# PieterBecking/so100-mujoco-rl

Measured on AMD Instinct MI355X. Metric: env steps/sec at 4096 envs/GPU, Env01 PPO rollout, higher is better.
Workload: dtype f32; 1 GPU; env01_free: Env01 x 4096 envs/GPU, frame_skip 16, contact disabled, no constraint solver (BASELINE.json configs[1]), SB3-MlpPolicy-shaped rollout (persistent policy), randomized resets, staggered episodes; envs_per_gpu=4096, rollout_chunk=64, parallelism=single GPU

## Files before the change

so100_mujoco_rl_amd/csrc/so100_kernels.hpp:

```cpp
#pragma once
#include <hip/hip_runtime.h>
#include <stdint.h>
#include <stdio.h>
#include <string.h>
#include <stdlib.h>
#include <new>
#include "../../include/so100_sim.h"
#include "so100_task.hpp"
#include "so100_policy.hpp"

namespace so100 {
template <int KIND, int FL = -1> __device__ __forceinline__ void load_env_state(const float* __restrict__ S, int n, int env, EnvState& e) {
#define X(name, member, kind, group) \
    if constexpr (uses_group<KIND, FL>(group)) { const float w_ = S[(size_t)SF_##name*n + env]; \
        if constexpr (#kind[0] == 'i') e.member = __float_as_int(w_); else e.member = w_; }
    SO100_STATE_FIELDS(X)
#undef X
}
template <typename M> __device__ __forceinline__ float as_word(M v) {
    if constexpr (sizeof(M) == 4 && !__is_floating_point(M)) return __int_as_float((int)v); else return (float)v;
}
template <int KIND, int FL = -1> __device__ __forceinline__ void store_env_state(float* __restrict__ S, int n, int env, const EnvState& e) {
#define X(name, member, kind, group) \
    if constexpr (uses_group<KIND, FL>(group)) S[(size_t)SF_##name*n + env] = as_word(e.member);
// ... 38 lines not shown
    store_env_state<KIND, FL>(io.state, p.n, env, e);
#pragma unroll
    for (int i = 0; i < OD; i++) io.obs[(size_t)env*OD + i] = obs[i];
    io.rew[env] = r.reward;
    if (io.rollout_row) {
        io.rollout_row[(size_t)env*(OD + ROW_EXTRA) + OD + ROW_REWARD] = r.reward;
        io.rollout_row[(size_t)env*(OD + ROW_EXTRA) + OD + ROW_DONE] = done_code(r.done, r.trunc_only);
    }
    io.done[env] = r.done ? 1 : 0;
    io.trunc[env] = r.trunc_only ? 1 : 0;
    if (r.done) {
        if (io.tobs) {
#pragma unroll
            for (int i = 0; i < OD; i++) io.tobs[(size_t)env*OD + i] = tobs[i];
        }
        if (io.ep_ret) io.ep_ret[env] = r.ep_return;
        if (io.ep_len) io.ep_len[env] = r.ep_length;
    }
}

template <int KIND, int FL>
__global__ void __launch_bounds__(256) so100_step_mw(SimParams p, StepPtrs io) {
    constexpr bool PADS = FL < 0 || (FL & (int)F_ANY_CONTACT) != 0;
    constexpr bool LINKS = FL < 0 || (FL & (int)F_ANY_LINKS) != 0;
    __shared__ float xq[PADS ? 24 : 18][64];
    __shared__ float xc[24][64];
    __shared__ float xb[6][64];
    __shared__ float cbuf[PADS ? MAXC*CF*64 : 1];
    __shared__ float xa[PADS ? 15 : 1][64];
    __shared__ float xk[PADS ? 12 : 1][64];
    __shared__ float xm[PADS ? 21 : 1][64];
    __shared__ unsigned char pbuf[PADS ? MAXC*64 : 1];
    __shared__ float xw[PADS ? 36 : 1][64];
    if (FL >= 0) p.flags = (unsigned)FL;
    const int lane = threadIdx.x & 63;
    const int wave = __builtin_amdgcn_readfirstlane(threadIdx.x >> 6);
    const int env = blockIdx.x*p.epw + lane;
    const bool live = lane < p.epw && env < p.n;
    constexpr int OD = obs_dim<KIND>();
    EnvState e; StepCtx ctx{}; float u[8] = {}; float cstale[3] = {};
    const float* inj = (io.inject && live) ? io.inject + (size_t)env*SO100_NINJECT : nullptr;
    if (wave == 0) {
        if (live) load_env_state<KIND, FL>(io.state, p.n, env, e); else idle_lane_state(e);
        float a[6];
#pragma unroll
        for (int i = 0; i < 6; i++) a[i] = live ? io.act[(size_t)env*6 + i] : 0.0f;
        draw8(p, p.env_id_offset + (uint32_t)env, (uint32_t)e.rngc, 0, inj, u);
        e.rngc++;
        env_step_pre<KIND>(e, a, u, p, ctx);
    }
    Arm<float> A; Prof prof_;
    const PhaseLds lds{ xq, xc, xb, cbuf, xa, xk, xm, pbuf, PADS ? xw : nullptr };
    ContactMemo memo;
    physics_phase_mw<PADS, LINKS, !PADS && FL != 7, !PADS && FL != 7, !PADS && FL != 7>(p, wave, lane, e, ctx.ctrl, cstale, A, lds, memo, prof_, [](int) {}, [&]() {
        ctx = StepCtx{};
#pragma unroll
        for (int k = 0; k < 8; k++) u[k] = 0.0f;
    });
    if (wave != 0 || !live) return;
    e.nsub += p.frame_skip;
    TaskPoses<float> P;
    task_poses<float, !PADS && FL != 7>(A.s, A.c, !reach_kind<KIND>(), P);
    float obs[OD], tobs[OD]; bool term;
    const float reward = env_step_post<KIND>(e, ctx, u, P, cstale, obs, term);
    const StepResult r = env_step_finish<KIND>(e, reward, term, p, p.env_id_offset + (uint32_t)env, inj, io.start_tab, obs, tobs);
    if constexpr (PADS) e.cload &= 0xFFFF;
    store_env_state<KIND, FL>(io.state, p.n, env, e);
#pragma unroll
    for (int i = 0; i < OD; i++) io.obs[(size_t)env*OD + i] = obs[i];
    io.rew[env] = r.reward;
    if (io.rollout_row) {
        io.rollout_row[(size_t)env*(OD + ROW_EXTRA) + OD + ROW_REWARD] = r.reward;
        io.rollout_row[(size_t)env*(OD + ROW_EXTRA) + OD + ROW_DONE] = done_code(r.done, r.trunc_only);
    }
    io.done[env] = r.done ? 1 : 0;
    io.trunc[env] = r.trunc_only ? 1 : 0;
    if (r.done) {
        if (io.tobs) {
#pragma unroll
            for (int i = 0; i < OD; i++) io.tobs[(size_t)env*OD + i] = tobs[i];
        }
        if (io.ep_ret) io.ep_ret[env] = r.ep_return;
        if (io.ep_len) io.ep_len[env] = r.ep_length;
    }
}

template <int KIND>
__global__ void __launch_bounds__(WG) so100_reset_masked(SimParams p, float* state, const float* start_tab,
                                                         const uint8_t* mask, const float* inject, float* obs_out) {
    const int env = blockIdx.x*WG + threadIdx.x;
    if (env >= p.n) return;
    if (mask && !mask[env]) return;
    EnvState e;
    load_env_state<KIND>(state, p.n, env, e);
    float u[8];
    const float* inj = inject ? inject + (size_t)env*SO100_NINJECT : nullptr;
    draw8(p, p.env_id_offset + (uint32_t)env, (uint32_t)e.rngc, 1, inj, u);
    e.rngc++;
    constexpr int OD = obs_dim<KIND>();
    float obs[OD];
    env_reset<KIND>(e, u, start_tab, obs);
    store_env_state<KIND>(state, p.n, env, e);
    if (obs_out) {
#pragma unroll
        for (int i = 0; i < OD; i++) obs_out[(size_t)env*OD + i] = obs[i];
    }
}

template <int KIND>
__global__ void __launch_bounds__(WG) so100_init_state(int n, float* state) {
    const int env = blockIdx.x*WG + threadIdx.x;
    if (env >= n) return;
    for (int f = 0; f < SF_COUNT; f++) state[(size_t)f*n + env] = 0.0f;
    EnvState e;
    env_init<KIND>(e);
    store_env_state<KIND>(state, n, env, e);
}


constexpr int MW_MAX_ENVS = 16384;
inline dim3 grid_for(int n) { return dim3((unsigned)((n + WG - 1)/WG)); }

struct RolloutPtrs { float* obs; float* rew; uint8_t* done; uint8_t* trunc; float* tobs; float* ep_ret; int32_t* ep_len; };

template <int KIND> struct KindOps {
    static hipError_t step(const SimParams& prm, const StepPtrs& io, hipStream_t st);
    static hipError_t reset(const SimParams& prm, float* state, const float* start_tab, const uint8_t* mask, const float* inject, float* obs, hipStream_t st);
    static hipError_t init(int n, float* state);
    static hipError_t rollout(const SimParams& prm, float* state, const float* start_tab, const RolloutPtrs& io, const PolicyWeights& pw, const RolloutArgs& ra, hipStream_t st);
#ifdef SO100_ROLLOUT_PROF
    static int prof_read(long long* out48);
    static int prof_read_wg(long long* wg4096, int* env32768);
    static int prof_read_hist(unsigned long long* hist48, int reset);
#endif
};
#ifdef SO100_ROLLOUT_PROF
template <int KIND> int KindOps<KIND>::prof_read(long long* out48) {
    return hipMemcpyFromSymbol(out48, HIP_SYMBOL(so100_prof), sizeof(long long)*48) == hipSuccess ? 0 : -1;
}
template <int KIND> int KindOps<KIND>::prof_read_hist(unsigned long long* h, int reset) {
    if (hipMemcpyFromSymbol(h, HIP_SYMBOL(so100_prof_hist), sizeof(unsigned long long)*48) != hipSuccess) return -1;
    if (reset) { unsigned long long z[48] = {}; if (hipMemcpyToSymbol(HIP_SYMBOL(so100_prof_hist), z, sizeof z) != hipSuccess) return -1; }
    return 0;
}
template <int KIND> int KindOps<KIND>::prof_read_wg(long long* wg, int* env) {
    if (hipMemcpyFromSymbol(wg, HIP_SYMBOL(so100_prof_wg), sizeof(long long)*4096) != hipSuccess) return -1;
    return hipMemcpyFromSymbol(env, HIP_SYMBOL(so100_prof_env), sizeof(int)*32768) == hipSuccess ? 0 : -1;
}
#endif

template <int KIND> hipError_t KindOps<KIND>::step(const SimParams& prm, const StepPtrs& io, hipStream_t st) {
    const bool mw = prm.n <= prm.mw_max;
    const dim3 g = mw ? dim3((unsigned)((prm.n + prm.epw - 1)/prm.epw)) : grid_for(prm.n), b(mw ? 256 : WG);
#define SO100_STEP(FLV) do { if (mw) hipLaunchKernelGGL((so100_step_mw<KIND, FLV>), g, b, 0, st, prm, io); \
                             else    hipLaunchKernelGGL((so100_step_fused<KIND, FLV>), g, b, 0, st, prm, io); } while (0)
#define SO100_STEP_ROWS(FLV) do { if (!mw && prm.n >= DENSE_MIN_ENVS) hipLaunchKernelGGL((so100_step_fused<KIND, FLV, true>), g, b, 0, st, prm, io); \
                                  else SO100_STEP(FLV); } while (0)
    switch (prm.flags) {
    case SO100_F_CUBE_PINNED: SO100_STEP(SO100_F_CUBE_PINNED); break;
    case SO100_F_FRICTIONLOSS | SO100_F_LIMITS | SO100_F_CUBE_PINNED: SO100_STEP_ROWS(SO100_F_FRICTIONLOSS | SO100_F_LIMITS | SO100_F_CUBE_PINNED); break;
    case SO100_F_NOPADS: SO100_STEP_ROWS(SO100_F_NOPADS); break;
    case SO100_F_REFERENCE: SO100_STEP(SO100_F_REFERENCE); break;
    case SO100_F_CONTACT5: if constexpr (reach_kind<KIND>()) { SO100_STEP(SO100_F_CONTACT5); } else { SO100_STEP(-1); } break;
    default: SO100_STEP(-1); break;
    }
#undef SO100_STEP_ROWS
#undef SO100_STEP
    return hipGetLastError();
}
template <int KIND> hipError_t KindOps<KIND>::reset(const SimParams& prm, float* state, const float* start_tab, const uint8_t* mask, const float* inject, float* obs, hipStream_t st) {
    hipLaunchKernelGGL(so100_reset_masked<KIND>, grid_for(prm.n), dim3(WG), 0, st, prm, state, start_tab, mask, inject, obs);
    return hipGetLastError();
}
template <int KIND> hipError_t KindOps<KIND>::init(int n, float* state) {
    hipLaunchKernelGGL(so100_init_state<KIND>, grid_for(n), dim3(WG), 0, nullptr, n, state);
    const hipError_t e = hipGetLastError();
    return e != hipSuccess ? e : hipDeviceSynchronize();
}
template <int KIND> hipError_t KindOps<KIND>::rollout(const SimParams& prm, float* state, const float* start_tab, const RolloutPtrs& io, const PolicyWeights& pw, const RolloutArgs& ra, hipStream_t st) {
    const dim3 grid((unsigned)((prm.n + prm.epw - 1)/prm.epw));
#define SO100_RL(FLV) hipLaunchKernelGGL((so100_rollout_fused<KIND, FLV, 4>), grid, dim3(256), 0, st, prm, state, start_tab, \
        io.obs, io.rew, io.done, io.trunc, io.tobs, io.ep_ret, io.ep_len, pw, ra)
    if (prm.flags == SO100_F_CUBE_PINNED) {
        if (prm.epw <= 32) hipLaunchKernelGGL((so100_rollout_fused<KIND, SO100_F_CUBE_PINNED, 4, 32>), grid, dim3(256), 0, st, prm, state, start_tab,
                                              io.obs, io.rew, io.done, io.trunc, io.tobs, io.ep_ret, io.ep_len, pw, ra);
        else SO100_RL(SO100_F_CUBE_PINNED);
    }
    else if (prm.flags == SO100_F_NOPADS) SO100_RL(SO100_F_NOPADS);
    else if (prm.flags == SO100_F_REFERENCE) SO100_RL(SO100_F_REFERENCE);
    else if (prm.flags == SO100_F_CONTACT5 && reach_kind<KIND>()) { if constexpr (reach_kind<KIND>()) SO100_RL(SO100_F_CONTACT5); }
    else SO100_RL(-1);
// ... 6 lines not shown
```

so100_mujoco_rl_amd/csrc/so100_rollout.hpp:

```cpp
#pragma once
#include "so100_policy.hpp"

namespace so100 {

struct RolloutArgs {
    float* buf;
    int32_t T;
    uint32_t step_counter0;
    const float* obs_in;
    float* tobs_chunk;
    const int32_t* slot_env;
};

typedef float f32x16 __attribute__((ext_vector_type(16)));

#ifdef SO100_ROLLOUT_PROF
__device__ long long so100_prof[48];
__device__ long long so100_prof_wg[1024*4];
__device__ int so100_prof_env[16384*2];
__device__ unsigned long long so100_prof_hist[48];
struct Prof {
    long long t[12] = {}, c = __builtin_readcyclecounter();
    int work = 0, insub = 0, sub = 0;
    __device__ __forceinline__ void substep_stats(bool solved, bool first_of_env) {
        const int f = sub & 255, s = (sub >> 8) & 255, g = (sub >> 16) & 255, l = (sub >> 24) & 255;
        work += f + s + g + l;
        int cost = solved ? 970*f + 140*s + 520*g + 300*l : 0, fmaxl = solved ? f : 0;
        const unsigned long long m = __ballot(solved && first_of_env);
        int best = cost, bf = fmaxl;
#pragma unroll
        for (int d = 32; d >= 1; d >>= 1) { const int oc = __shfl_xor(best, d, 64), of = __shfl_xor(bf, d, 64); if (oc > best) { best = oc; bf = of; } }
        if (solved && first_of_env) {
            atomicAdd(&so100_prof_hist[33], (unsigned long long)f); atomicAdd(&so100_prof_hist[34], (unsigned long long)s);
            atomicAdd(&so100_prof_hist[35], (unsigned long long)g); atomicAdd(&so100_prof_hist[36], (unsigned long long)l);
            atomicAdd(&so100_prof_hist[40], (unsigned long long)cost);
        }
        if ((threadIdx.x & 63) == 0) {
            const int ne = __popcll(m);
            atomicAdd(&so100_prof_hist[16 + (ne > 16 ? 16 : ne)], 1ull); atomicAdd(&so100_prof_hist[39], 1ull);
            if (m) { atomicAdd(&so100_prof_hist[bf > 15 ? 15 : bf], 1ull); atomicAdd(&so100_prof_hist[37], (unsigned long long)best); atomicAdd(&so100_prof_hist[38], 1ull); }
        }
        sub = 0;
    }
    __device__ __forceinline__ void mark(int slot) { const long long n = __builtin_readcyclecounter(); t[slot] += n - c; c = n; }
    __device__ __forceinline__ void flush(int base, bool who) const { if (who) for (int i = 0; i < 12; i++) so100_prof[base + i] = t[i]; }
    __device__ __forceinline__ void flush_wg(int wave, int lane, int env, bool live) const {
        if (blockIdx.x < 1024 && lane == 0) {
            long long tot = 0; for (int i = 0; i < 12; i++) tot += t[i];
            if (wave == 0) { so100_prof_wg[blockIdx.x*4 + 0] = tot; so100_prof_wg[blockIdx.x*4 + 3] = t[8]; }
            if (wave == 3) { so100_prof_wg[blockIdx.x*4 + 1] = t[4] + t[10]; so100_prof_wg[blockIdx.x*4 + 2] = t[6] + t[11]; }
        }
        if (wave == 3 && live && env < 16384) { so100_prof_env[2*env] = work; so100_prof_env[2*env + 1] = insub; }
    }
};
#define SO100_PROF_WORK (&prof_.sub)
#define SO100_PROF_INSUB() (prof_.insub++)
#else
struct Prof {
    __device__ __forceinline__ void substep_stats(bool, bool) {}
    __device__ __forceinline__ void mark(int) {}
    __device__ __forceinline__ void flush(int, bool) const {}
    __device__ __forceinline__ void flush_wg(int, int, int, bool) const {}
};
#define SO100_PROF_WORK nullptr
#define SO100_PROF_INSUB() ((void)0)
#endif
#define SO100_PROF_DECL Prof prof_;
#define SO100_PROF(slot) prof_.mark(slot)
#define SO100_PROF_FLUSH(base) prof_.flush((base), blockIdx.x == 0 && lane == 0)

struct PhaseLds { float (*xq)[64]; float (*xc)[64]; float (*xb)[64]; float* cbuf; float (*xa)[64]; float (*xk)[64]; float (*xm)[64]; unsigned char* pbuf; float (*xw)[64]; };
struct ContactMemo { int zones = -1, prev_n = 0; };

constexpr int XC_POS = 0, XC_QUAT = 3, XC_VEL = 7, XC_WARM = 13, XC_ANTIGRAV = 19, XC_STALE = 20;
__device__ __forceinline__ void cube_to_lds(float (*xc)[64], int col, const Cube<float>& c) {
#pragma unroll
    for (int i = 0; i < 3; i++) xc[XC_POS + i][col] = c.pos[i];
#pragma unroll
    for (int i = 0; i < 4; i++) xc[XC_QUAT + i][col] = c.quat[i];
#pragma unroll
    for (int i = 0; i < 6; i++) { xc[XC_VEL + i][col] = c.vel[i]; xc[XC_WARM + i][col] = c.warm[i]; }
}
__device__ __forceinline__ void cube_from_lds(float (*xc)[64], int col, Cube<float>& c) {
#pragma unroll
    for (int i = 0; i < 3; i++) c.pos[i] = xc[XC_POS + i][col];
#pragma unroll
    for (int i = 0; i < 4; i++) c.quat[i] = xc[XC_QUAT + i][col];
#pragma unroll
    for (int i = 0; i < 6; i++) { c.vel[i] = xc[XC_VEL + i][col]; c.warm[i] = xc[XC_WARM + i][col]; }
}

template <bool PADS, bool LINKS, bool PK, bool LOCAL, bool Z, class Hook, class Forget>
__device__ __forceinline__ void physics_phase_mw(const SimParams& p, int wave, int lane, EnvState& e, float ctrl[6], float cstale[3],
                                                 Arm<float>& A, const PhaseLds& L, ContactMemo& memo, Prof& prof_, Hook after_first_barrier, Forget forget_caller_state) {
    float (*xq)[64] = L.xq; float (*xc)[64] = L.xc; float (*xb)[64] = L.xb; float (*xa)[64] = L.xa; float (*xk)[64] = L.xk; float (*xm)[64] = L.xm;
    float dq[6] = { 0.0f, 0.0f, 0.0f, 0.0f, 0.0f, 0.0f };
    const bool cube_live = (p.flags & F_CUBE_PINNED) == 0u;
    const bool pads = PADS && (p.flags & F_ANY_CONTACT) != 0u;
    const bool padcube = PADS && (p.flags & F_ARM_CUBE) != 0u && cube_live;
    Cube<float> cb; CubePrep<float> cprep;
    float applied[3] = { 0.0f, 0.0f, 0.0f };
    memo = ContactMemo{};
    const int np3 = 64/p.epw, sh3 = np3 == 4 ? 2 : np3 == 2 ? 1 : 0;
    const int el = lane >> sh3, part3 = lane & (np3 - 1);
    if (wave == 0) {
        e.res = 0.0f; e.cstat = 0; e.csig = 0;
        if (pads) {
#pragma unroll
            for (int i = 0; i < 6; i++) { xk[i][lane] = ctrl[i]; xk[6 + i][lane] = e.aw[i]; }
        }
    }
    if (cube_live) {
        if (wave == 0) {
            cube_to_lds(xc, lane, e.cube);
            xc[XC_ANTIGRAV][lane] = (e.bits & B_ANTIGRAV) ? (float)(so100g::CUBE_MASS*so100g::GRAVITY) : 0.0f;
        }
        __syncthreads();
        if (wave == 2) {
            cube_from_lds(xc, lane, cb);
            applied[2] = xc[XC_ANTIGRAV][lane];
        }
    } else {
        if (wave == 0) { cstale[0] = e.cube.pos[0]; cstale[1] = e.cube.pos[1]; cstale[2] = e.cube.pos[2]; }
        if (pads) __syncthreads();
    }
    if (pads && wave == 3) { xa[12][lane] = 0.0f; xa[14][lane] = 0.0f; }
#pragma unroll 1
    for (int sub = 0; sub < p.frame_skip; sub++) {
        if (wave == 0) {
            if (sub == 0) arm_trig<float>(e.q, A); else arm_trig_update<float, PK>(e.q, dq, A);
#pragma unroll
            for (int i = 0; i < 6; i++) { xq[i][lane] = A.s[i]; xq[6 + i][lane] = A.c[i]; xq[12 + i][lane] = e.v[i]; }
            if (pads) {
#pragma unroll
                for (int i = 0; i < 6; i++) xq[18 + i][lane] = e.q[i];
            }
            SO100_PROF(2);
        }
        if (padcube && wave == 2 && sub > 0) cube_to_lds(xc, lane, cb);
        __syncthreads();
        SO100_PROF(3);
        after_first_barrier(sub);
        WorldFK<float> W3; Arm<float> A3; ContactsLds<float> cs3{ L.cbuf, el, L.pbuf, part3, np3 };
        cs3.prev_n = memo.prev_n;
        float Rc3[9] = { 1.0f, 0.0f, 0.0f, 0.0f, 1.0f, 0.0f, 0.0f, 0.0f, 1.0f }, cpos3[3] = { 0.0f, 0.0f, 0.0f };
        bool coupled3 = false, any3 = false;
        static_assert(!LOCAL || !PADS, "the loop-local factor is written for the variants without pad contacts (nothing publishes M)");
        Arm<float> Fl; Arm<float>& F = LOCAL ? Fl : A;
        if (LOCAL && wave == 0) {
#pragma unroll
            for (int i = 0; i < 6; i++) { F.s[i] = A.s[i]; F.c[i] = A.c[i]; }
            arm_mass<float, PK, Z>(F);
            arm_factor<float>(p.flags, F);
            SO100_PROF(4);
        } else if (LOCAL && wave == 1) {
            Arm<float> R; float v1[6];
#pragma unroll
            for (int i = 0; i < 6; i++) { R.s[i] = xq[i][lane]; R.c[i] = xq[6 + i][lane]; v1[i] = xq[12 + i][lane]; }
            arm_bias<float, PK, Z>(v1, R);
#pragma unroll
            for (int i = 0; i < 6; i++) xb[i][lane] = R.bias[i];
            SO100_PROF(4);
        } else if (wave == 1) {
            float v1[6], q1[6] = { 0.0f, 0.0f, 0.0f, 0.0f, 0.0f, 0.0f }, c1[6] = { 0.0f, 0.0f, 0.0f, 0.0f, 0.0f, 0.0f };
#pragma unroll
            for (int i = 0; i < 6; i++) { A.s[i] = xq[i][lane]; A.c[i] = xq[6 + i][lane]; v1[i] = xq[12 + i][lane]; }
            if (pads) {
#pragma unroll
                for (int i = 0; i < 6; i++) { q1[i] = xq[18 + i][lane]; c1[i] = xk[i][lane]; }
            }
            arm_bias<float, PK, Z>(v1, A);
#pragma unroll
            for (int i = 0; i < 6; i++) xb[i][lane] = A.bias[i];
            if (pads) {
                float t1[6]; ArmRows<float> r1;
                arm_tau<float>(q1, v1, c1, A, t1);
                arm_row_consts<float>(q1, v1, p.flags, r1);
#pragma unroll
                for (int i = 0; i < 6; i++) { xa[i][lane] = t1[i]; xa[6 + i][lane] = r1.clv[i]; xq[18 + i][lane] = r1.sg[i]*r1.Dl[i]; }
            }
            SO100_PROF(4);
        } else if (wave == 0) {
            arm_mass<float, PK, Z>(A);
            if (pads) {
#pragma unroll
                for (int i = 0; i < 21; i++) xm[i][lane] = A.M[i];
            }
            arm_factor<float>(p.flags, A);
            SO100_PROF(4);
        } else if (wave == 2 && cube_live) {
            if (sub == p.frame_skip - 1) { xc[XC_STALE][lane] = cb.pos[0]; xc[XC_STALE + 1][lane] = cb.pos[1]; xc[XC_STALE + 2][lane] = cb.pos[2]; }
            cube_prepare<float>(cb, applied, p.flags, cprep);
            SO100_PROF(4);
        } else if (wave == 3 && pads) {
            float v3[6];
// ... 255 lines not shown
        __syncthreads();
        if (wave == 0 && live) {
            float lp = 0.0f;
#pragma unroll
            for (int a = 0; a < 6; a++) {
                const float ls = hd[HD_LOG_STD + a], e = xn[a][lane];
                const float act = __builtin_fmaf(__builtin_expf(ls), e, xmean[a][lane]);
                lp += -0.5f*e*e - ls - 0.9189385332046727f;
                io.act_env[(size_t)env*6 + a] = tclamp(act, -1.0f, 1.0f);
                if (io.act_raw) io.act_raw[(size_t)env*6 + a] = act;
                if (io.rollout_row) io.rollout_row[(size_t)env*(OD + ROW_EXTRA) + OD + ROW_ACT + a] = act;
            }
            if (io.logp) io.logp[env] = lp;
            if (io.rollout_row) io.rollout_row[(size_t)env*(OD + ROW_EXTRA) + OD + ROW_LOGP] = lp;
        } else if (wave == 1 && live && io.rollout_row) {
#pragma unroll
            for (int k = 0; k < OD; k++) io.rollout_row[(size_t)env*(OD + ROW_EXTRA) + k] = oxt[lane][k];
        }
    }
}

template <int KIND, int FL, int NW, int ROWS = 64>
__global__ void __launch_bounds__(64*NW) so100_rollout_fused(SimParams p, float* __restrict__ state, const float* start_tab,
                                                             float* obs_out, float* rew_out, uint8_t* done_out, uint8_t* trunc_out,
                                                             float* tobs_out, float* ep_ret_out, int32_t* ep_len_out,
                                                             PolicyWeights w, RolloutArgs ra) {
    static_assert(NW == 4, "one wave per SIMD: (tower, row tile) per wave");
    static_assert(ROWS == 64 || ROWS == 32, "envs per workgroup the policy phase is tiled for");
    constexpr bool HALF = ROWS == 32;
    constexpr int OD = obs_dim<KIND>();
    constexpr int ODP = policy_odp(OD);
    constexpr int LD = POLICY_LD;
    __shared__ __attribute__((aligned(16))) float hd[HD_WORDS];
    __shared__ float oxt[64][ODP + 1];
    constexpr int HB = 2*2*64*LD;
    __shared__ float pool[HB + 6*64];
    float (*h1t)[64][LD] = reinterpret_cast<float (*)[64][LD]>(pool);
    float (*h2t)[64][LD] = reinterpret_cast<float (*)[64][LD]>(pool + 2*64*LD);
    float (*xmean)[64] = reinterpret_cast<float (*)[64]>(pool + HB);
    float (*xm)[64] = reinterpret_cast<float (*)[64]>(pool + MAXC*CF*64);
    static_assert(HB + 6*64 >= MAXC*CF*64 + 21*64, "contact records + mass matrix must fit under the policy phase's images");
    constexpr bool XW = FL >= 0 && (FL & (int)F_PADS_CUBE) == 0 && (FL & (int)F_PADS_FLOOR) != 0;
    static_assert(!XW || MAXPADC*CF*64 + 36*64 <= MAXC*CF*64, "joint frames must fit in the unused tail of the contact store");
    float (*xw)[64] = XW ? reinterpret_cast<float (*)[64]>(pool + MAXPADC*CF*64) : nullptr;
    constexpr bool PADS = FL < 0 || (FL & (int)F_ANY_CONTACT) != 0;
    constexpr bool LINKS = FL < 0 || (FL & (int)F_ANY_LINKS) != 0;
    __shared__ float xa[PADS ? 15 : 1][64];
    __shared__ float xk[PADS ? 12 : 1][64];
    __shared__ float xn[6][64];
    __shared__ float xq[PADS ? 24 : 18][64];
    __shared__ float xc[24][64];
    __shared__ float xb[6][64];
    __shared__ unsigned char pbuf[PADS ? MAXC*64 : 1];
    ContactMemo memo;
    if (FL >= 0) p.flags = (unsigned)FL;
    const int lane = threadIdx.x & 63;
    const int wave = __builtin_amdgcn_readfirstlane(threadIdx.x >> 6);
    const int slot = blockIdx.x*p.epw + lane;
    const int env = lane < p.epw ? (ra.slot_env ? ra.slot_env[slot] : (slot < p.n ? slot : -1)) : -1;
    const bool live = env >= 0;
    const int tower = wave >> 1, rt = wave & 1;
    const int lj = lane & 31, lh = lane >> 5;
    const float* W1 = tower ? w.vf_w0 : w.pi_w0; const float* W2 = tower ? w.vf_w1 : w.pi_w1;
    const float* Bi1 = tower ? w.vf_b0 : w.pi_b0; const float* Bi2 = tower ? w.vf_b1 : w.pi_b1;
    constexpr bool W2_LDS = FL != (int)F_CUBE_PINNED;
    static_assert(!HALF || !W2_LDS, "the 32-row tiling exists for the contact-disabled variant");
    constexpr int NCT = HALF ? 1 : 2;
    float bw1[NCT][ODP/2], bw2[NCT][W2_LDS ? 1 : 32], b1v[NCT], b2v[NCT];
    __shared__ float w2s[W2_LDS ? 4 : 1][2][32][W2_LDS ? 64 : 1];
#pragma unroll
    for (int ct = 0; ct < NCT; ct++) {
        const int unit = 32*(HALF ? rt : ct) + lj;
        b1v[ct] = Bi1[unit]; b2v[ct] = Bi2[unit];
#pragma unroll
        for (int s2 = 0; s2 < ODP/2; s2++) { const int k = 2*s2 + lh; bw1[ct][s2] = k < OD ? W1[unit*OD + k] : 0.0f; }
#pragma unroll
        for (int s2 = 0; s2 < 32; s2++) { if constexpr (W2_LDS) w2s[wave][ct][s2][lane] = W2[unit*64 + 2*s2 + lh]; else bw2[ct][s2] = W2[unit*64 + 2*s2 + lh]; }
    }
    if (wave == NW - 1) {
        for (int i = lane; i < 6*64; i += 64) hd[HD_MU_W + i] = w.mu_w[i];
        hd[HD_V_W + lane] = w.v_w[lane];
        if (lane < 6) { hd[HD_MU_B + lane] = w.mu_b[lane]; hd[HD_LOG_STD + lane] = w.log_std[lane]; }
        if (lane == 0) hd[HD_V_B] = w.v_b[0];
    }
    EnvState e;
    if (wave == 0) {
        if (live) load_env_state<KIND, FL>(state, p.n, env, e); else idle_lane_state(e);
#pragma unroll
        for (int k = 0; k < ODP; k++) oxt[lane][k] = (live && k < OD) ? ra.obs_in[(size_t)env*OD + k] : 0.0f;
    }
    if (wave == 3 && ra.T > 0) {
        float eps[8];
        policy_noise(p.env_id_offset + (uint32_t)env, ra.step_counter0, p.seed_lo, p.seed_hi, eps);
#pragma unroll
        for (int a = 0; a < 6; a++) xn[a][lane] = eps[a];
    }
    __syncthreads();
    StepResult last{}; float last_obs[OD];
    StepCtx ctx{}; float ustep[8] = {}; float cstale[3] = {};
    SO100_PROF_DECL
#pragma unroll 1
    for (int t = 0; t < ra.T; t++) {
        SO100_PROF(7);
        if constexpr (HALF) {
            f32x16 acc;
#pragma unroll
            for (int r = 0; r < 16; r++) acc[r] = b1v[0];
#pragma unroll
            for (int s2 = 0; s2 < ODP/2; s2++) acc = __builtin_amdgcn_mfma_f32_32x32x2f32(oxt[lj][2*s2 + lh], bw1[0][s2], acc, 0, 0, 0);
#pragma unroll
            for (int r = 0; r < 16; r++) h1t[tower][(r & 3) + 8*(r >> 2) + 4*lh][32*rt + lj] = fast_tanh(acc[r]);
        } else {
            f32x16 acc0, acc1;
#pragma unroll
            for (int r = 0; r < 16; r++) { acc0[r] = b1v[0]; acc1[r] = b1v[1]; }
#pragma unroll
            for (int s2 = 0; s2 < ODP/2; s2++) {
                const float a = oxt[32*rt + lj][2*s2 + lh];
                acc0 = __builtin_amdgcn_mfma_f32_32x32x2f32(a, bw1[0][s2], acc0, 0, 0, 0);
                acc1 = __builtin_amdgcn_mfma_f32_32x32x2f32(a, bw1[1][s2], acc1, 0, 0, 0);
            }
#pragma unroll
            for (int r = 0; r < 16; r++) {
                const int row = 32*rt + (r & 3) + 8*(r >> 2) + 4*lh;
                h1t[tower][row][lj] = fast_tanh(acc0[r]); h1t[tower][row][32 + lj] = fast_tanh(acc1[r]);
            }
        }
        __syncthreads();
        if constexpr (HALF) {
            f32x16 acc;
#pragma unroll
            for (int r = 0; r < 16; r++) acc[r] = b2v[0];
#pragma unroll
            for (int s2 = 0; s2 < 32; s2++) acc = __builtin_amdgcn_mfma_f32_32x32x2f32(h1t[tower][lj][2*s2 + lh], bw2[0][s2], acc, 0, 0, 0);
#pragma unroll
            for (int r = 0; r < 16; r++) h2t[tower][(r & 3) + 8*(r >> 2) + 4*lh][32*rt + lj] = fast_tanh(acc[r]);
        } else {
            f32x16 acc0, acc1;
#pragma unroll
            for (int r = 0; r < 16; r++) { acc0[r] = b2v[0]; acc1[r] = b2v[1]; }
#pragma unroll
            for (int s2 = 0; s2 < 32; s2++) {
                const float a = h1t[tower][32*rt + lj][2*s2 + lh];
                float b0, b1;
                if constexpr (W2_LDS) { b0 = w2s[wave][0][s2][lane]; b1 = w2s[wave][1][s2][lane]; } else { b0 = bw2[0][s2]; b1 = bw2[1][s2]; }
                acc0 = __builtin_amdgcn_mfma_f32_32x32x2f32(a, b0, acc0, 0, 0, 0);
                acc1 = __builtin_amdgcn_mfma_f32_32x32x2f32(a, b1, acc1, 0, 0, 0);
            }
#pragma unroll
            for (int r = 0; r < 16; r++) {
                const int row = 32*rt + (r & 3) + 8*(r >> 2) + 4*lh;
                h2t[tower][row][lj] = fast_tanh(acc0[r]); h2t[tower][row][32 + lj] = fast_tanh(acc1[r]);
            }
        }
        __syncthreads();
        SO100_PROF(0);
        float* row = ra.buf + ((size_t)t*p.n + (size_t)env)*(OD + ROW_EXTRA);
        if (wave != 2) {
            const int a0 = wave == 0 ? 0 : (wave == 1 ? 2 : 4);
            float m0 = hd[HD_MU_B + a0], m1 = hd[HD_MU_B + a0 + 1];
#pragma unroll 4
            for (int k = 0; k < 64; k += 4) {
                const float x0 = h2t[0][lane][k], x1 = h2t[0][lane][k+1], x2 = h2t[0][lane][k+2], x3 = h2t[0][lane][k+3];
                const float4 w0 = *reinterpret_cast<const float4*>(&hd[a0*64 + k]);
                const float4 w1 = *reinterpret_cast<const float4*>(&hd[(a0 + 1)*64 + k]);
                m0 = __builtin_fmaf(w0.x, x0, m0); m0 = __builtin_fmaf(w0.y, x1, m0); m0 = __builtin_fmaf(w0.z, x2, m0); m0 = __builtin_fmaf(w0.w, x3, m0);
                m1 = __builtin_fmaf(w1.x, x0, m1); m1 = __builtin_fmaf(w1.y, x1, m1); m1 = __builtin_fmaf(w1.z, x2, m1); m1 = __builtin_fmaf(w1.w, x3, m1);
            }
            xmean[a0][lane] = m0; xmean[a0 + 1][lane] = m1;
        } else {
            float v = hd[HD_V_B];
#pragma unroll 8
            for (int k = 0; k < 64; k++) v = __builtin_fmaf(hd[HD_V_W + k], h2t[1][lane][k], v);
            if (live) row[OD + ROW_VALUE] = v;
        }
        __syncthreads();
        if (wave == 0) {
            float mean[6], eps[6];
#pragma unroll
            for (int a = 0; a < 6; a++) { mean[a] = xmean[a][lane]; eps[a] = xn[a][lane]; }
            float act[6], lp = 0.0f;
#pragma unroll
            for (int a = 0; a < 6; a++) {
                const float ls = hd[HD_LOG_STD + a];
                const float raw = __builtin_fmaf(__builtin_expf(ls), eps[a], mean[a]);
                lp += -0.5f*eps[a]*eps[a] - ls - 0.9189385332046727f;
                act[a] = live ? tclamp(raw, -1.0f, 1.0f) : 0.0f;
                if (live) row[OD + ROW_ACT + a] = raw;
            }
            if (live) {
#pragma unroll
                for (int k = 0; k < OD; k++) row[k] = oxt[lane][k];
                row[OD + ROW_LOGP] = lp;
            }
            draw8(p, p.env_id_offset + (uint32_t)env, (uint32_t)e.rngc, 0, nullptr, ustep);
            e.rngc++;
            env_step_pre<KIND>(e, act, ustep, p, ctx);
            SO100_PROF(1);
        }
        {
            Arm<float> A;
            const PhaseLds lds{ xq, xc, xb, pool, xa, xk, xm, pbuf, xw };
            constexpr bool PKF = !PADS && FL != 7;
            physics_phase_mw<PADS, LINKS, PKF, PKF && KIND != 3 && KIND != 4, PKF>(p, wave, lane, e, ctx.ctrl, cstale, A, lds, memo, prof_, [&](int sub) {
                if (wave == 3 && sub == 0 && t + 1 < ra.T) {
                    float eps[8];
                    policy_noise(p.env_id_offset + (uint32_t)env, ra.step_counter0 + (uint32_t)(t + 1), p.seed_lo, p.seed_hi, eps);
#pragma unroll
                    for (int a = 0; a < 6; a++) xn[a][lane] = eps[a];
                }
            }, [&]() {
                ctx = StepCtx{}; last = StepResult{};
#pragma unroll
                for (int k = 0; k < 8; k++) ustep[k] = 0.0f;
#pragma unroll
                for (int k = 0; k < OD; k++) last_obs[k] = 0.0f;
            });
            if (wave == 0) {
                e.nsub += p.frame_skip;
                TaskPoses<float> P;
                task_poses<float, PKF>(A.s, A.c, !reach_kind<KIND>(), P);
                float obs[OD], tobs[OD]; bool term;
                const float reward = env_step_post<KIND>(e, ctx, ustep, P, cstale, obs, term);
                const StepResult r = env_step_finish<KIND>(e, reward, term, p, p.env_id_offset + (uint32_t)env, nullptr, start_tab, obs, tobs);
#pragma unroll
                for (int k = 0; k < OD; k++) { oxt[lane][k] = obs[k]; last_obs[k] = obs[k]; }
                last = r;
                if (live) {
                    row[OD + ROW_REWARD] = r.reward; row[OD + ROW_DONE] = done_code(r.done, r.trunc_only);
                    if (r.done) {
                        if (ra.tobs_chunk) {
#pragma unroll
                            for (int k = 0; k < OD; k++) ra.tobs_chunk[((size_t)t*p.n + (size_t)env)*OD + k] = tobs[k];
                        }
                        if (tobs_out) {
#pragma unroll
                            for (int k = 0; k < OD; k++) tobs_out[(size_t)env*OD + k] = tobs[k];
                        }
                        if (ep_ret_out) ep_ret_out[env] = r.ep_return;
                        if (ep_len_out) ep_len_out[env] = r.ep_length;
                    }
                }
            }
        }
        __syncthreads();
    }
    SO100_PROF_FLUSH(12*wave);
    {
        const int np = 64/p.epw, e3 = blockIdx.x*p.epw + lane/np;
        if (wave == 3) prof_.flush_wg(wave, lane, e3, (lane % np) == 0 && e3 < p.n); else prof_.flush_wg(wave, lane, env, live);
    }
    if (wave == 0 && live) {
        if constexpr (PADS) {
            const unsigned hist = (unsigned)e.cload & 0xFFFFu, now = (unsigned)e.cload >> 16;
            e.cload = (int)(((hist < CLOAD_MAX ? hist : CLOAD_MAX) + (now < CLOAD_MAX ? now : CLOAD_MAX)) >> 1);
        }
        store_env_state<KIND, FL>(state, p.n, env, e);
        if (ra.T > 0) {
#pragma unroll
            for (int k = 0; k < OD; k++) obs_out[(size_t)env*OD + k] = last_obs[k];
            rew_out[env] = last.reward; done_out[env] = last.done ? 1 : 0; trunc_out[env] = last.trunc_only ? 1 : 0;
        }
    }
}

}
```

so100_mujoco_rl_amd/csrc/so100_sim.hip:

```cpp
#include "so100_kernels.hpp"
#include "so100_balance.hpp"
#include "so100_render.hpp"
#include "so100_policy_tensors.h"
#include "so100_host.hpp"

namespace so100 {
extern template struct KindOps<1>; extern template struct KindOps<2>; extern template struct KindOps<3>;
extern template struct KindOps<4>; extern template struct KindOps<5>; extern template struct KindOps<6>;
}

namespace {

using namespace so100;

const char* const kFieldNames[] = {
#define X(name, member, kind, group) #name,
    SO100_STATE_FIELDS(X)
#undef X
};

#include "so100_start_positions.inc"

}

// ... 40 lines not shown
    s->prm.max_episode_steps = cfg->max_episode_steps;
    s->prm.seed_lo = (uint32_t)cfg->seed; s->prm.seed_hi = (uint32_t)(cfg->seed >> 32);
    s->prm.env_id_offset = cfg->env_id_offset;
    hipDeviceProp_t prop;
    int cus = 256;
    if (hipGetDeviceProperties(&prop, cfg->device) == hipSuccess && prop.multiProcessorCount > 0) cus = prop.multiProcessorCount;
    s->prm.epw = choose_envs_per_workgroup(*cfg, cus);
    s->prm.mw_max = MW_MAX_ENVS;
    if (const char* ov = getenv("SO100_MW_MAX_ENVS")) { const long v = atol(ov); if (v >= 0) s->prm.mw_max = (int32_t)(v > (1L << 30) ? (1L << 30) : v); }
    const size_t bytes = (size_t)SF_COUNT*(size_t)cfg->num_envs*sizeof(float);
    if (hipMalloc(&s->state, bytes) != hipSuccess) return fail(SO100_E_NOMEM, "so100_create: hipMalloc of %ld bytes failed", (long)bytes);
    float tab[36*6];
    for (int i = 0; i < 36; i++) for (int j = 0; j < 6; j++) tab[6*i + j] = (float)SO100_VALID_START_POSITIONS[i][j];
    if (hipMalloc(&s->start_tab, sizeof tab) != hipSuccess || hipMemcpy(s->start_tab, tab, sizeof tab, hipMemcpyHostToDevice) != hipSuccess)
        return fail(SO100_E_NOMEM, "so100_create: start table upload failed");
    const char* bal = getenv("SO100_BALANCE");
    const bool pads = (cfg->flags & (SO100_F_PADS_FLOOR | SO100_F_PADS_CUBE | SO100_F_LINKS_FLOOR | SO100_F_LINKS_CUBE)) != 0;
    if (pads && cfg->num_envs <= BALANCE_MAX_ENVS && !(bal && atoi(bal) == 0)) {
        const size_t slots = (size_t)((cfg->num_envs + s->prm.epw - 1)/s->prm.epw)*(size_t)s->prm.epw;
        if (hipMalloc(&s->slot_env, slots*sizeof(int32_t)) != hipSuccess) return fail(SO100_E_NOMEM, "so100_create: hipMalloc of the slot map failed");
    }
    HIP_TRY(DISPATCH_KIND(cfg->env_kind, init)(s->prm.n, s->state), SO100_E_LAUNCH, "so100_create: ");
    return 0;
}

struct RowCopy { int row, rows; const void* user; };
int move_rows(so100_sim* s, const char* fn, bool to_state, std::initializer_list<RowCopy> copies, void* stream) {
    SO100_ON_DEVICE(s->cfg.device, fn);
    const size_t n = (size_t)s->prm.n;
    for (const RowCopy& c : copies) {
        float* mine = s->state + (size_t)c.row*n;
        const size_t bytes = (size_t)c.rows*n*sizeof(float);
        if (!c.user) HIP_TRY(hipMemsetAsync(mine, 0, bytes, (hipStream_t)stream), SO100_E_LAUNCH);
        else if (to_state) HIP_TRY(hipMemcpyAsync(mine, c.user, bytes, hipMemcpyDeviceToDevice, (hipStream_t)stream), SO100_E_LAUNCH);
        else HIP_TRY(hipMemcpyAsync(const_cast<void*>(c.user), mine, bytes, hipMemcpyDeviceToDevice, (hipStream_t)stream), SO100_E_LAUNCH);
    }
    return 0;
}
}

extern "C" {

int so100_abi_version(void) { return SO100_ABI_VERSION; }
int so100_obs_dim(int32_t kind) { return (kind == 1 || kind == 2 || kind == 6) ? 15 : (kind >= 3 && kind <= 5) ? 8 : -1; }
int so100_num_state_fields(void) { return SF_COUNT; }
int so100_state_field_index(const char* name) {
    if (!name) return -1;
    for (int i = 0; i < SF_COUNT; i++) if (strcmp(kFieldNames[i], name) == 0) return i;
    return -1;
}
const char* so100_state_field_name(int32_t field) { return (field >= 0 && field < SF_COUNT) ? kFieldNames[field] : nullptr; }
const char* so100_last_error(void) { return g_last_error; }
#ifdef SO100_ROLLOUT_PROF
int so100_prof_read(int kind, long long* out48) { return DISPATCH_KIND(kind, prof_read)(out48); }
int so100_prof_read_wg(int kind, long long* wg4096, int* env32768) { return DISPATCH_KIND(kind, prof_read_wg)(wg4096, env32768); }
int so100_prof_read_hist(int kind, unsigned long long* hist48, int reset) { return DISPATCH_KIND(kind, prof_read_hist)(hist48, reset); }
#endif

int so100_create(const so100_config* cfg, so100_sim** out) {
    if (!cfg || !out) return fail(SO100_E_INVALID, "so100_create: null argument");
    *out = nullptr;
    if (cfg->env_kind < 1 || cfg->env_kind > 6) return fail(SO100_E_INVALID, "so100_create: env_kind must be 1..6");
    if (cfg->num_envs < 1) return fail(SO100_E_INVALID, "so100_create: num_envs must be >= 1");
    if (cfg->solver_iters < 1 || cfg->solver_iters > 64) return fail(SO100_E_INVALID, "so100_create: solver_iters must be in 1..64");
    if (cfg->contact_iters < 1 || cfg->contact_iters > 64) return fail(SO100_E_INVALID, "so100_create: contact_iters must be in 1..64");
    if (cfg->frame_skip < 1 || cfg->frame_skip > 1024) return fail(SO100_E_INVALID, "so100_create: frame_skip must be in 1..1024");
    if (cfg->max_episode_steps < 0) return fail(SO100_E_INVALID, "so100_create: max_episode_steps must be >= 0");
    if (cfg->flags & ~(SO100_F_FRICTIONLOSS | SO100_F_LIMITS | SO100_F_FLOOR | SO100_F_CUBE_PINNED | SO100_F_PADS_FLOOR | SO100_F_PADS_CUBE | SO100_F_LINKS_FLOOR | SO100_F_LINKS_CUBE))
        return fail(SO100_E_INVALID, "so100_create: unknown flag bits");
    if ((cfg->flags & (SO100_F_PADS_CUBE | SO100_F_LINKS_CUBE)) && (cfg->flags & SO100_F_CUBE_PINNED))
        return fail(SO100_E_INVALID, "so100_create: SO100_F_PADS_CUBE / SO100_F_LINKS_CUBE need a dynamic cube (not SO100_F_CUBE_PINNED)");
    if (cfg->envs_per_workgroup != 0 && cfg->envs_per_workgroup != 16 && cfg->envs_per_workgroup != 32 && cfg->envs_per_workgroup != 64)
        return fail(SO100_E_INVALID, "so100_create: envs_per_workgroup must be 0 (automatic), 16, 32 or 64");
    if ((cfg->flags & SO100_F_FLOOR) && (cfg->flags & SO100_F_CUBE_PINNED))
        return fail(SO100_E_INVALID, "so100_create: SO100_F_FLOOR and SO100_F_CUBE_PINNED are mutually exclusive");
    int ndev = 0;
    if (hipGetDeviceCount(&ndev) != hipSuccess || ndev < 1)
        return fail(SO100_E_NODEVICE, "so100_create: no HIP device available (this library has no CPU fallback)");
    if (cfg->device < 0 || cfg->device >= ndev) return fail(SO100_E_INVALID, "so100_create: device ordinal out of range");
    SO100_ON_DEVICE(cfg->device, "so100_create");
    so100_sim* s = new (std::nothrow) so100_sim();
    if (!s) return fail(SO100_E_NOMEM, "so100_create: out of host memory");
    s->cfg = *cfg;
    const int rc = create_on_device(s);
    if (rc != 0) { so100_destroy(s); return rc; }
    *out = s;
    return 0;
}

int so100_envs_per_workgroup(const so100_sim* s) { return s ? s->prm.epw : SO100_E_INVALID; }

void so100_destroy(so100_sim* s) {
    if (!s) return;
    DeviceGuard g(s->cfg.device);
    if (s->state) (void)hipFree(s->state);
    if (s->start_tab) (void)hipFree(s->start_tab);
    if (s->slot_env) (void)hipFree(s->slot_env);
    if (s->render_scene) (void)hipFree(s->render_scene);
    delete s;
}

int so100_reset(so100_sim* s, const uint8_t* mask_dev, const float* inject_dev, float* obs_dev, void* stream) {
    if (!s) return fail(SO100_E_INVALID, "so100_reset: null handle");
    SO100_ON_DEVICE(s->cfg.device, "so100_reset");
    HIP_TRY(DISPATCH_KIND(s->cfg.env_kind, reset)(s->prm, s->state, s->start_tab, mask_dev, inject_dev, obs_dev, (hipStream_t)stream), SO100_E_LAUNCH);
    return 0;
}
// ... 117 lines not shown
```

Baseline: 151.7 million env-steps/s.

## Precompute first-substep bias and mass factor on idle waves during policy sampling

For the pinned-cube configuration without pad contacts, the env's q and v are mirrored into LDS. While wave 0 samples actions, waves 1 and 2 compute trig, bias forces and the LDL mass factorization for the first physics substep, and wave 3 writes the observation row. The physics loop then starts from that precomputed factor: wave 0 does only the solve and integrate for substep 0, and the loop begins at substep 1. This moves dependent-chain work off the serial critical path, at the cost of extra LDS arrays, one more barrier and a duplicated first-substep code path. Profiling slots are widened to match.

```diff
diff --git a/so100_mujoco_rl_amd/csrc/so100_kernels.hpp b/so100_mujoco_rl_amd/csrc/so100_kernels.hpp
--- a/so100_mujoco_rl_amd/csrc/so100_kernels.hpp
+++ b/so100_mujoco_rl_amd/csrc/so100_kernels.hpp
@@ -114,7 +114,7 @@
     Arm<float> A; Prof prof_;
     const PhaseLds lds{ xq, xc, xb, cbuf, xa, xk, xm, pbuf, PADS ? xw : nullptr };
     ContactMemo memo;
-    physics_phase_mw<PADS, LINKS, !PADS && FL != 7, !PADS && FL != 7, !PADS && FL != 7>(p, wave, lane, e, ctx.ctrl, cstale, A, lds, memo, prof_, [](int) {}, [&]() {
+    physics_phase_mw<PADS, LINKS, !PADS && FL != 7, !PADS && FL != 7, !PADS && FL != 7, false>(p, wave, lane, e, ctx.ctrl, cstale, A, lds, memo, prof_, [](int) {}, [&]() {
         ctx = StepCtx{};
 #pragma unroll
         for (int k = 0; k < 8; k++) u[k] = 0.0f;
@@ -191,14 +191,14 @@
     static hipError_t init(int n, float* state);
     static hipError_t rollout(const SimParams& prm, float* state, const float* start_tab, const RolloutPtrs& io, const PolicyWeights& pw, const RolloutArgs& ra, hipStream_t st);
 #ifdef SO100_ROLLOUT_PROF
-    static int prof_read(long long* out48);
+    static int prof_read(long long* out64);
     static int prof_read_wg(long long* wg4096, int* env32768);
     static int prof_read_hist(unsigned long long* hist48, int reset);
 #endif
 };
 #ifdef SO100_ROLLOUT_PROF
-template <int KIND> int KindOps<KIND>::prof_read(long long* out48) {
-    return hipMemcpyFromSymbol(out48, HIP_SYMBOL(so100_prof), sizeof(long long)*48) == hipSuccess ? 0 : -1;
+template <int KIND> int KindOps<KIND>::prof_read(long long* out64) {
+    return hipMemcpyFromSymbol(out64, HIP_SYMBOL(so100_prof), sizeof(long long)*64) == hipSuccess ? 0 : -1;
 }
 template <int KIND> int KindOps<KIND>::prof_read_hist(unsigned long long* h, int reset) {
     if (hipMemcpyFromSymbol(h, HIP_SYMBOL(so100_prof_hist), sizeof(unsigned long long)*48) != hipSuccess) return -1;
diff --git a/so100_mujoco_rl_amd/csrc/so100_rollout.hpp b/so100_mujoco_rl_amd/csrc/so100_rollout.hpp
--- a/so100_mujoco_rl_amd/csrc/so100_rollout.hpp
+++ b/so100_mujoco_rl_amd/csrc/so100_rollout.hpp
@@ -15,12 +15,12 @@
 typedef float f32x16 __attribute__((ext_vector_type(16)));
 
 #ifdef SO100_ROLLOUT_PROF
-__device__ long long so100_prof[48];
+__device__ long long so100_prof[64];
 __device__ long long so100_prof_wg[1024*4];
 __device__ int so100_prof_env[16384*2];
 __device__ unsigned long long so100_prof_hist[48];
 struct Prof {
-    long long t[12] = {}, c = __builtin_readcyclecounter();
+    long long t[16] = {}, c = __builtin_readcyclecounter();
     int work = 0, insub = 0, sub = 0;
     __device__ __forceinline__ void substep_stats(bool solved, bool first_of_env) {
         const int f = sub & 255, s = (sub >> 8) & 255, g = (sub >> 16) & 255, l = (sub >> 24) & 255;
@@ -43,10 +43,10 @@
         sub = 0;
     }
     __device__ __forceinline__ void mark(int slot) { const long long n = __builtin_readcyclecounter(); t[slot] += n - c; c = n; }
-    __device__ __forceinline__ void flush(int base, bool who) const { if (who) for (int i = 0; i < 12; i++) so100_prof[base + i] = t[i]; }
+    __device__ __forceinline__ void flush(int base, bool who) const { if (who) for (int i = 0; i < 16; i++) so100_prof[base + i] = t[i]; }
     __device__ __forceinline__ void flush_wg(int wave, int lane, int env, bool live) const {
         if (blockIdx.x < 1024 && lane == 0) {
-            long long tot = 0; for (int i = 0; i < 12; i++) tot += t[i];
+            long long tot = 0; for (int i = 0; i < 16; i++) tot += t[i];
             if (wave == 0) { so100_prof_wg[blockIdx.x*4 + 0] = tot; so100_prof_wg[blockIdx.x*4 + 3] = t[8]; }
             if (wave == 3) { so100_prof_wg[blockIdx.x*4 + 1] = t[4] + t[10]; so100_prof_wg[blockIdx.x*4 + 2] = t[6] + t[11]; }
         }
@@ -90,7 +90,7 @@
     for (int i = 0; i < 6; i++) { c.vel[i] = xc[XC_VEL + i][col]; c.warm[i] = xc[XC_WARM + i][col]; }
 }
 
-template <bool PADS, bool LINKS, bool PK, bool LOCAL, bool Z, class Hook, class Forget>
+template <bool PADS, bool LINKS, bool PK, bool LOCAL, bool Z, bool PRE, class Hook, class Forget>
 __device__ __forceinline__ void physics_phase_mw(const SimParams& p, int wave, int lane, EnvState& e, float ctrl[6], float cstale[3],
                                                  Arm<float>& A, const PhaseLds& L, ContactMemo& memo, Prof& prof_, Hook after_first_barrier, Forget forget_caller_state) {
     float (*xq)[64] = L.xq; float (*xc)[64] = L.xc; float (*xb)[64] = L.xb; float (*xa)[64] = L.xa; float (*xk)[64] = L.xk; float (*xm)[64] = L.xm;
@@ -125,10 +125,38 @@
         if (pads) __syncthreads();
     }
     if (pads && wave == 3) { xa[12][lane] = 0.0f; xa[14][lane] = 0.0f; }
+    static_assert(!PRE || (LOCAL && !PADS), "the pre-computed first half is written for the loop-local factor without pad contacts");
+    if constexpr (PRE) {
+        __syncthreads();
+        SO100_PROF(15);
+        if (p.frame_skip == 1) after_first_barrier(0);
+        if (wave == 0) {
+            Arm<float> F0; float tau[6], acc0[6];
+#pragma unroll
+            for (int i = 0; i < 6; i++) { A.s[i] = xq[i][lane]; A.c[i] = xq[6 + i][lane]; F0.bias[i] = xb[i][lane]; F0.Dinv[i] = xm[15 + i][lane]; }
+#pragma unroll
+            for (int i = 1; i < 6; i++)
+#pragma unroll
+                for (int k = 0; k < i; k++) F0.M[SO100_TRI(i, k)] = xm[SO100_TRI(i - 1, k)][lane];
+#pragma unroll
+            for (int i = 0; i < 6; i++) {
+                const float u = tclamp(ctrl[i], (float)-so100g::ACT_CTRL, (float)so100g::ACT_CTRL), ku = (float)so100g::ACT_KP*u;
+                float f = __builtin_fmaf(-(float)so100g::ACT_KP, e.q[i], ku);
+                f = __builtin_fmaf(-(float)so100g::ACT_KV[i], e.v[i], f);
+                tau[i] = tclamp(f, (float)-so100g::ACT_FORCE, (float)so100g::ACT_FORCE) - F0.bias[i];
+            }
+#pragma unroll
+            for (int i = 0; i < 6; i++) acc0[i] = tau[i];
+            ldl6_solve<float>(F0.M, F0.Dinv, acc0);
+            SO100_PROF(6);
+            arm_integrate<float>(e.q, e.v, e.qc, acc0, dq);
+            SO100_PROF(9);
+        }
+    }
 #pragma unroll 1
-    for (int sub = 0; sub < p.frame_skip; sub++) {
+    for (int sub = PRE ? 1 : 0; sub < p.frame_skip; sub++) {
         if (wave == 0) {
-            if (sub == 0) arm_trig<float>(e.q, A); else arm_trig_update<float, PK>(e.q, dq, A);
+            if (!PRE && sub == 0) arm_trig<float>(e.q, A); else arm_trig_update<float, PK>(e.q, dq, A);
 #pragma unroll
             for (int i = 0; i < 6; i++) { xq[i][lane] = A.s[i]; xq[6 + i][lane] = A.c[i]; xq[12 + i][lane] = e.v[i]; }
             if (pads) {
@@ -140,7 +168,7 @@
         if (padcube && wave == 2 && sub > 0) cube_to_lds(xc, lane, cb);
         __syncthreads();
         SO100_PROF(3);
-        after_first_barrier(sub);
+        after_first_barrier(PRE && sub == 1 ? 0 : sub);
         WorldFK<float> W3; Arm<float> A3; ContactsLds<float> cs3{ L.cbuf, el, L.pbuf, part3, np3 };
         cs3.prev_n = memo.prev_n;
         float Rc3[9] = { 1.0f, 0.0f, 0.0f, 0.0f, 1.0f, 0.0f, 0.0f, 0.0f, 1.0f }, cpos3[3] = { 0.0f, 0.0f, 0.0f };
@@ -502,6 +530,10 @@
     __shared__ float xc[24][64];
     __shared__ float xb[6][64];
     __shared__ unsigned char pbuf[PADS ? MAXC*64 : 1];
+    constexpr bool PKF = !PADS && FL != 7, LOCALF = PKF && KIND != 3 && KIND != 4;
+    constexpr bool PRE = LOCALF && FL == (int)F_CUBE_PINNED;
+    __shared__ float xs[PRE ? 12 : 1][64];
+    __shared__ float xf[PRE ? 21 : 1][64];
     ContactMemo memo;
     if (FL >= 0) p.flags = (unsigned)FL;
     const int lane = threadIdx.x & 63;
@@ -538,6 +570,10 @@
         if (live) load_env_state<KIND, FL>(state, p.n, env, e); else idle_lane_state(e);
 #pragma unroll
         for (int k = 0; k < ODP; k++) oxt[lane][k] = (live && k < OD) ? ra.obs_in[(size_t)env*OD + k] : 0.0f;
+        if constexpr (PRE) {
+#pragma unroll
+            for (int i = 0; i < 6; i++) { xs[i][lane] = e.q[i]; xs[6 + i][lane] = e.v[i]; }
+        }
     }
     if (wave == 3 && ra.T > 0) {
         float eps[8];
@@ -625,6 +661,7 @@
             if (live) row[OD + ROW_VALUE] = v;
         }
         __syncthreads();
+        SO100_PROF(12);
         if (wave == 0) {
             float mean[6], eps[6];
 #pragma unroll
@@ -639,20 +676,53 @@
                 if (live) row[OD + ROW_ACT + a] = raw;
             }
             if (live) {
-#pragma unroll
-                for (int k = 0; k < OD; k++) row[k] = oxt[lane][k];
+                if constexpr (!PRE) {
+#pragma unroll
+                    for (int k = 0; k < OD; k++) row[k] = oxt[lane][k];
+                }
                 row[OD + ROW_LOGP] = lp;
             }
             draw8(p, p.env_id_offset + (uint32_t)env, (uint32_t)e.rngc, 0, nullptr, ustep);
             e.rngc++;
             env_step_pre<KIND>(e, act, ustep, p, ctx);
             SO100_PROF(1);
+        } else if constexpr (PRE) {
+          if (wave == 1) {
+            Arm<float> R; float q1[6], v1[6];
+#pragma unroll
+            for (int i = 0; i < 6; i++) { q1[i] = xs[i][lane]; v1[i] = xs[6 + i][lane]; }
+            arm_trig<float>(q1, R);
+#pragma unroll
+            for (int i = 0; i < 6; i++) { xq[i][lane] = R.s[i]; xq[6 + i][lane] = R.c[i]; }
+            SO100_PROF(13);
+            arm_bias<float, PKF, PKF>(v1, R);
+#pragma unroll
+            for (int i = 0; i < 6; i++) xb[i][lane] = R.bias[i];
+            SO100_PROF(14);
+          } else if (wave == 2) {
+            Arm<float> F; float q2[6];
+#pragma unroll
+            for (int i = 0; i < 6; i++) q2[i] = xs[i][lane];
+            arm_trig<float>(q2, F);
+            SO100_PROF(13);
+            arm_mass<float, PKF, PKF>(F);
+            arm_factor<float>(p.flags, F);
+#pragma unroll
+            for (int i = 1; i < 6; i++)
+#pragma unroll
+                for (int k = 0; k < i; k++) xf[SO100_TRI(i - 1, k)][lane] = F.M[SO100_TRI(i, k)];
+#pragma unroll
+            for (int i = 0; i < 6; i++) xf[15 + i][lane] = F.Dinv[i];
+            SO100_PROF(14);
+          } else if (live) {
+#pragma unroll
+            for (int k = 0; k < OD; k++) row[k] = oxt[lane][k];
+          }
         }
         {
             Arm<float> A;
-            const PhaseLds lds{ xq, xc, xb, pool, xa, xk, xm, pbuf, xw };
-            constexpr bool PKF = !PADS && FL != 7;
-            physics_phase_mw<PADS, LINKS, PKF, PKF && KIND != 3 && KIND != 4, PKF>(p, wave, lane, e, ctx.ctrl, cstale, A, lds, memo, prof_, [&](int sub) {
+            const PhaseLds lds{ xq, xc, xb, pool, xa, xk, PRE ? xf : xm, pbuf, xw };
+            physics_phase_mw<PADS, LINKS, PKF, LOCALF, PKF, PRE>(p, wave, lane, e, ctx.ctrl, cstale, A, lds, memo, prof_, [&](int sub) {
                 if (wave == 3 && sub == 0 && t + 1 < ra.T) {
                     float eps[8];
                     policy_noise(p.env_id_offset + (uint32_t)env, ra.step_counter0 + (uint32_t)(t + 1), p.seed_lo, p.seed_hi, eps);
@@ -675,6 +745,10 @@
                 const StepResult r = env_step_finish<KIND>(e, reward, term, p, p.env_id_offset + (uint32_t)env, nullptr, start_tab, obs, tobs);
 #pragma unroll
                 for (int k = 0; k < OD; k++) { oxt[lane][k] = obs[k]; last_obs[k] = obs[k]; }
+                if constexpr (PRE) {
+#pragma unroll
+                    for (int i = 0; i < 6; i++) { xs[i][lane] = e.q[i]; xs[6 + i][lane] = e.v[i]; }
+                }
                 last = r;
                 if (live) {
                     row[OD + ROW_REWARD] = r.reward; row[OD + ROW_DONE] = done_code(r.done, r.trunc_only);
@@ -695,7 +769,7 @@
         }
         __syncthreads();
     }
-    SO100_PROF_FLUSH(12*wave);
+    SO100_PROF_FLUSH(16*wave);
     {
         const int np = 64/p.epw, e3 = blockIdx.x*p.epw + lane/np;
         if (wave == 3) prof_.flush_wg(wave, lane, e3, (lane % np) == 0 && e3 < p.n); else prof_.flush_wg(wave, lane, env, live);
diff --git a/so100_mujoco_rl_amd/csrc/so100_sim.hip b/so100_mujoco_rl_amd/csrc/so100_sim.hip
--- a/so100_mujoco_rl_amd/csrc/so100_sim.hip
+++ b/so100_mujoco_rl_amd/csrc/so100_sim.hip
@@ -116,7 +116,7 @@
 const char* so100_state_field_name(int32_t field) { return (field >= 0 && field < SF_COUNT) ? kFieldNames[field] : nullptr; }
 const char* so100_last_error(void) { return g_last_error; }
 #ifdef SO100_ROLLOUT_PROF
-int so100_prof_read(int kind, long long* out48) { return DISPATCH_KIND(kind, prof_read)(out48); }
+int so100_prof_read(int kind, long long* out64) { return DISPATCH_KIND(kind, prof_read)(out64); }
 int so100_prof_read_wg(int kind, long long* wg4096, int* env32768) { return DISPATCH_KIND(kind, prof_read_wg)(wg4096, env32768); }
 int so100_prof_read_hist(int kind, unsigned long long* hist48, int reset) { return DISPATCH_KIND(kind, prof_read_hist)(hist48, reset); }
 #endif
```

Measured after the change: 157.9 million env-steps/s, median of 6. 4.0% higher.
